# yzGuu830/efficient-speech-codec

Hardware: AMD Instinct MI355X
Metric: audio-seconds/sec encode+decode, ESC-Base 9kbps 3s@16kHz (higher is better)
Workload: dtype f32 (fp32 storage and accumulation everywhere; the K = C contractions of the MLPs, of the attention's Q / K / V projections, of PatchMerge / PatchSplit and of the de-embedding run on the fp16 matrix cores with every fp32 operand split into two fp16 terms under power-of-two scales (range-safe by cons

## Files before the change

efficient-speech-codec_amd/csrc/fused_attn.h:

```cpp
#pragma once
#include <hip/hip_runtime.h>
#include <type_traits>
#include "gemm_engine.h"
#include "gemm_bf16.h"
#include "split_terms.h"

namespace escx {

constexpr int attn_x3_ks(int CP) { return (CP + 31) / 32; }
constexpr int attn_x3_tf(int CP, int NT = 3) { return NT * attn_x3_ks(CP) > CP / 16 ? NT * attn_x3_ks(CP) : CP / 16; }
__device__ __forceinline__ void attn_split3(const float (&v)[8], bf16x8& t0, bf16x8& t1, bf16x8& t2) {
#pragma clang fp contract(off)
#pragma unroll
    for (int e = 0; e < 8; ++e) {
        const __bf16 a1 = (__bf16)v[e];
        const float r1 = v[e] - (float)a1;
        const __bf16 a2 = (__bf16)r1;
        const float r2 = r1 - (float)a2;
        t0[e] = a1; t1[e] = a2; t2[e] = (__bf16)r2;
    }
}
__global__ __launch_bounds__(256) void attn_x3_pack_kernel(const f32x4* __restrict__ waf, bf16x8* __restrict__ out, bf16x8* __restrict__ tail, int n_tiles, int TPG, int KK, int KS, int TF, unsigned proj_mask, int NT = 3,
                                                           const float* __restrict__ gamma = nullptr, const float* __restrict__ beta = nullptr, int n_ln = 0, int C = 0,
                                                           const float* __restrict__ bqkv = nullptr, int n_bqkv = 0) {
    const int per_tile = (KS > KK ? KS : KK) * 64;
    const long long idx = (long long)blockIdx.x * 256 + threadIdx.x;
    if (idx >= (long long)n_tiles * per_tile) return;
    const int tile = (int)(idx / per_tile), r = (int)(idx - (long long)tile * per_tile), f = r >> 6, lane = r & 63;
    const f32x4* src = waf + (size_t)tile * KK * 64;
    bf16x8* dst = out + (size_t)tile * TF * 64;
    if ((proj_mask >> (tile % TPG)) & 1) {
        if (f < KK) {
            const f32x4 w = src[f * 64 + lane];
            if (NT == 2 && bqkv) {
                const float sc = x2_scale(reinterpret_cast<const unsigned*>(tail)[2]);
                const float v[8] = {w[0], w[1], w[2], w[3], 0.f, 0.f, 0.f, 0.f};
                bf16x8 t[2];
                split_terms<2>(v, t, sc);
                const f32x4 hi = __builtin_bit_cast(f32x4, t[0]), lo = __builtin_bit_cast(f32x4, t[1]);
                reinterpret_cast<f32x4*>(dst)[f * 64 + lane] = f32x4{hi[0], hi[1], lo[0], lo[1]};
            } else {
                reinterpret_cast<f32x4*>(dst)[f * 64 + lane] = w;
            }
        }
        return;
    }
    if (f >= KS) return;
    const int l15 = lane & 15, g = lane >> 4;
    float v[8];
#pragma unroll
    for (int e = 0; e < 8; ++e) {
        const int kk = 2 * f + (g >> 1), lgs = 2 * (g & 1) + (e >> 2);
        v[e] = kk < KK ? src[kk * 64 + 16 * lgs + l15][e & 3] : 0.f;
    }
    if (NT == 3) {
        bf16x8 t0, t1, t2;
        attn_split3(v, t0, t1, t2);
        dst[(f * 3 + 0) * 64 + lane] = t0; dst[(f * 3 + 1) * 64 + lane] = t1; dst[(f * 3 + 2) * 64 + lane] = t2;
    } else {
        const float sc = x2_scale(*reinterpret_cast<const unsigned*>(tail));
        bf16x8 t[2];
        split_terms<2>(v, t, sc);
        dst[(f * 2 + 0) * 64 + lane] = t[0]; dst[(f * 2 + 1) * 64 + lane] = t[1];
        if (idx == 0) {
            const float bx = gamma ? ln_out_bound(gamma, beta, n_ln, C) : 0.f;
            const float sx = gamma ? act_pow2_scale(bx) : 1.0f;
            float so = 1.0f;
            const unsigned* mxs = reinterpret_cast<const unsigned*>(tail);
            if (bqkv && gamma) {
                float mb = 0.f;
                for (int i = 0; i < n_bqkv; ++i) mb = fmaxf(mb, fabsf(bqkv[i]));
                so = act_pow2_scale((float)C * __uint_as_float(mxs[1]) * bx + mb);
            }
            float* o = reinterpret_cast<float*>(tail + 1); o[0] = (1.0f / sc) * (1.0f / sx); o[1] = sc * sx; o[2] = sx; o[3] = so;
            if (bqkv) { o[4] = (1.0f / x2_scale(mxs[2])) * (1.0f / so); o[5] = 0.f; o[6] = 0.f; o[7] = 0.f; }
        }
    }
}

struct AttnArgs {
    const float* src;
    float* dst;
    const float* gamma; const float* beta;
    const f32x4* wf;
    const float* bqkv;
    const float* bias_tab;
    const float* bproj;
    const int* map;
    int slots, tokens, n_windows, nWh, nWw, shifted, C, n_groups;
    float scale, eps;
    int GS; float* partial; int rows;
    unsigned long long* trace;
    float* tape_xn; float* tape_qkv; float* tape_o; int ldq, ldo, hdp, nH;
    const void* x3_wf;
    const float* x3_scale;
};

__device__ __forceinline__ f32x4 window_shift_mask(int l15, int lg, bool lastH, bool lastW) {
    const int qh = l15 >> 2, qw = l15 & 3;
    const int labq = 3 * (lastH ? (qh < 2 ? 1 : 2) : 0) + (lastW ? (qw < 2 ? 1 : 2) : 0);
    const int labkh = 3 * (lastH ? (lg < 2 ? 1 : 2) : 0);
    f32x4 m;
#pragma unroll
    for (int r = 0; r < 4; ++r) {
        const int labk = labkh + (lastW ? (r < 2 ? 1 : 2) : 0);
        m[r] = (labk != labq) ? -100.0f : 0.0f;
    }
    return m;
}

__device__ __forceinline__ f32x4 window_softmax(f32x4 s, f32x4 bias_row, f32x4 shift_mask, bool shifted) {
    s += bias_row;
    if (shifted) s += shift_mask;
    float mx = fmaxf(fmaxf(s[0], s[1]), fmaxf(s[2], s[3]));
    mx = max_groups(mx);
    const float ml = -mx * 1.44269504088896341f;
    f32x4 p;
#pragma unroll
    for (int r = 0; r < 4; ++r) p[r] = __builtin_amdgcn_exp2f(fmaf(s[r], 1.44269504088896341f, ml));
    float den = (p[0] + p[1]) + (p[2] + p[3]);
    den = sum_groups(den);
    const float inv = __builtin_amdgcn_rcpf(den);
#pragma unroll
    for (int r = 0; r < 4; ++r) p[r] *= inv;
    return p;
}

#ifndef ESCX_ATTN_OCC3
#define ESCX_ATTN_OCC3 160
#endif
template <int CP, int TMW> constexpr int attn_min_waves() { return (CP * TMW <= 96) ? 4 : ((CP * TMW <= ESCX_ATTN_OCC3) ? 3 : ((CP * TMW <= 192) ? 2 : 1)); }

template <int CP, int TMW, bool X3> constexpr int attn_min_waves_x() { return !X3 ? attn_min_waves<CP, TMW>() : ((CP * TMW <= 96) ? 3 : ((CP * TMW <= 160) ? 2 : 1)); }

template <int CP, int MODE, int TMW, int NW, bool X3, int NT> constexpr int attn_min_waves_f() { return (X3 && NT == 2 && NW == 8 && MODE == 0 && TMW == 1 && CP <= 96) ? 4 : attn_min_waves_x<CP, TMW, X3>(); }

template <int CP, int MODE, int UT, int TMW, int NW, bool TAPE = false, bool X3 = false, int NT = 3>
__global__ __launch_bounds__(64 * NW, (attn_min_waves_f<CP, MODE, TMW, NW, X3, NT>())) void attn_fused_kernel(AttnArgs a) {
    static_assert(!X3 || !TAPE, "the split-operand form exists for the plain inference instantiations");
    static_assert(NT == 3 || (NT == 2 && X3), "two fp16 terms: the split-operand instantiations");
#ifdef ESCX_ATTN_PRIO
    __builtin_amdgcn_s_setprio(ESCX_ATTN_PRIO);
#endif
    constexpr int KK = CP / 16;
    constexpr int TPG = (MODE == 2) ? 8 : 4;
    constexpr int NB = (MODE == 2) ? 6 : 3;
    static_assert(TPG % UT == 0, "stage size must divide the tiles of a head group");
    constexpr int KS = attn_x3_ks(CP);
    constexpr int TF = X3 ? attn_x3_tf(CP, NT) : KK;
    __shared__ f32x4 wbuf_static[X3 ? 1 : 2 * UT * KK * 64];
    extern __shared__ __attribute__((aligned(16))) f32x4 wbuf_dyn[];
    f32x4* const wbuf0 = X3 ? wbuf_dyn : wbuf_static;

    const int lane = threadIdx.x & 63;
    const int l15 = lane & 15, lg = lane >> 4;
    const int wave = __builtin_amdgcn_readfirstlane(threadIdx.x >> 6);
    const int GS = a.GS > 1 ? a.GS : 1;
    const int wgb = blockIdx.x / GS, gs = blockIdx.x - wgb * GS;
    const int g0 = gs * (a.n_groups / GS), g1 = g0 + a.n_groups / GS;
    const int win0 = (wgb * NW + wave) * TMW;
    const int n_stages = (g1 - g0) * (TPG / UT);
    const f32x4* wfb = (X3 ? reinterpret_cast<const f32x4*>(a.x3_wf) : a.wf) + (size_t)g0 * TPG * TF * 64;

    constexpr int NP = UT * TF, NPW = (NP + NW - 1) / NW;
    const f32x4* dma_src = wfb + lane;
    f32x4* dma_dst = wbuf0;
    int slot = 0;
    auto dma_slot = [&]() {
        if (slot < NPW) {
            int c = wave + slot * NW;
            if (NP % NW != 0) c = min(c, NP - 1);
            __builtin_amdgcn_global_load_lds((const void*)(dma_src + c * 64), (__attribute__((address_space(3))) void*)(dma_dst + c * 64), 16, 0, 0);
        }
        ++slot;
    };
#pragma unroll
    for (int i = 0; i < NPW; ++i) dma_slot();

    const int nW = a.nWh * a.nWw;
    f32x4 xf[X3 ? 1 : TMW][X3 ? 1 : KK];
    bf16x8 xs[X3 ? TMW : 1][NT][X3 ? KS : 1];
    float x2_dn = 1.f, x2_up = 1.f, x2_sx = 1.f, x2_so = 1.f;
    if constexpr (NT == 2) { x2_dn = a.x3_scale[0]; x2_up = a.x3_scale[1]; x2_sx = a.x3_scale[2]; x2_so = a.x3_scale[3]; }
    int tok[TMW];
    bool lastH[TMW], lastW[TMW];
#pragma unroll
    for (int t = 0; t < TMW; ++t) {
        const int win = win0 + t;
        tok[t] = -1; lastH[t] = false; lastW[t] = false;
        if (win < a.n_windows) {
            const int b = win / nW, wloc = win - b * nW;
            const int wh = wloc / a.nWw, ww = wloc - wh * a.nWw;
            lastH[t] = (wh == a.nWh - 1); lastW[t] = (ww == a.nWw - 1);
            const int tk = a.map[wloc * 16 + l15];
            if (tk >= 0) tok[t] = b * a.tokens + tk;
        }
        if constexpr (X3) {
            const float* xrow = a.src + (size_t)(tok[t] < 0 ? 0 : tok[t]) * CP;
            float xv[KS][8];
            float s = 0.f;
#pragma unroll
            for (int ks = 0; ks < KS; ++ks) {
                const int c0 = 32 * ks + 8 * lg;
                f32x4 v0 = zero4(), v1 = zero4();
                if (c0 < CP) { v0 = ld4(xrow + c0); v1 = ld4(xrow + c0 + 4); }
                if (tok[t] < 0) { v0 = zero4(); v1 = zero4(); }
#pragma unroll
                for (int e = 0; e < 4; ++e) { xv[ks][e] = v0[e]; xv[ks][4 + e] = v1[e]; s += v0[e]; s += v1[e]; }
            }
            s = sum_groups(s);
            const float mean = s / (float)a.C;
            float v = 0.f;
#pragma unroll
            for (int ks = 0; ks < KS; ++ks)
#pragma unroll
                for (int e = 0; e < 8; ++e) { const float d = xv[ks][e] - mean; v += d * d; }
            v = sum_groups(v) - (float)(32 * KS - a.C) * mean * mean;
            const float rstd = 1.0f / sqrtf(v / (float)a.C + a.eps);
#pragma unroll
            for (int ks = 0; ks < KS; ++ks) {
                const int c0 = 32 * ks + 8 * lg;
                f32x4 g0v = zero4(), g1v = zero4(), b0v = zero4(), b1v = zero4();
// ... 151 lines not shown
#pragma unroll
        for (int t = 0; t < TMW; ++t) { out[t] = init; o2[t] = zero4(); }
#pragma unroll
        for (int kk = 0; kk < KK; ++kk) {
            const f32x4 w = next_frag();
            if ((kk & 1) == 0) dma_pinned();
#pragma unroll
            for (int r = 0; r < 4; ++r)
#pragma unroll
                for (int t = 0; t < TMW; ++t) {
                    if (TMW == 1 && (r & 1)) o2[t] = __builtin_amdgcn_mfma_f32_16x16x4f32(w[r], xf[t][kk][r], o2[t], 0, 0, 0);
                    else out[t] = __builtin_amdgcn_mfma_f32_16x16x4f32(w[r], xf[t][kk][r], out[t], 0, 0, 0);
                }
            ESCX_SGB_MFMA(4 * TMW);
        }
        if (TMW == 1) out[0] += o2[0];
    };
    auto gemm_x_rows = [&](f32x4* out, f32x4 init) {
        if constexpr (X3) { gemm_x3(out, init, true); return; }
        f32x4 o2[TMW];
#pragma unroll
        for (int t = 0; t < TMW; ++t) { out[t] = init; o2[t] = zero4(); }
#pragma unroll
        for (int kk = 0; kk < KK; ++kk) {
            const f32x4 w = next_frag();
            if ((kk & 1) == 0) dma_pinned();
#pragma unroll
            for (int r = 0; r < 4; ++r)
#pragma unroll
                for (int t = 0; t < TMW; ++t) {
                    if (TMW == 1 && (r & 1)) o2[t] = __builtin_amdgcn_mfma_f32_16x16x4f32(xf[t][kk][r], w[r], o2[t], 0, 0, 0);
                    else out[t] = __builtin_amdgcn_mfma_f32_16x16x4f32(xf[t][kk][r], w[r], out[t], 0, 0, 0);
                }
            ESCX_SGB_MFMA(4 * TMW);
        }
        if (TMW == 1) out[0] += o2[0];
    };
    auto proj_accumulate = [&](const f32x4* o) {
        const f32x4* tb = wb + (size_t)(((tile - 1) % UT) * TF) * 64;
        if constexpr (X3 && NT == 2) {
            bf16x8 os[TMW][2];
#pragma unroll
            for (int t = 0; t < TMW; ++t) {
                const float v8[8] = {o[t][0], o[t][1], o[t][2], o[t][3], 0.f, 0.f, 0.f, 0.f};
                split_terms<2>(v8, os[t], x2_so);
            }
#pragma unroll
            for (int to = 0; to < KK; to += 2) {
                const f32x4 w = tb[to * 64], wn = (to + 1 < KK) ? tb[(to + 1) * 64] : zero4();
                dma_pinned();
                const bf16x8 wh = __builtin_bit_cast(bf16x8, f32x4{w[0], w[1], 0.f, 0.f}), wl = __builtin_bit_cast(bf16x8, f32x4{w[2], w[3], 0.f, 0.f});
                const bf16x8 wnh = __builtin_bit_cast(bf16x8, f32x4{wn[0], wn[1], 0.f, 0.f}), wnl = __builtin_bit_cast(bf16x8, f32x4{wn[2], wn[3], 0.f, 0.f});
#define ESCX_PJ2(WH, WL, TO) _Pragma("unroll") for (int t = 0; t < TMW; ++t) acc[TO][t] = mma_x<2>(WH, os[t][1], acc[TO][t]); \
                             _Pragma("unroll") for (int t = 0; t < TMW; ++t) acc[TO][t] = mma_x<2>(WL, os[t][0], acc[TO][t]); \
                             _Pragma("unroll") for (int t = 0; t < TMW; ++t) acc[TO][t] = mma_x<2>(WH, os[t][0], acc[TO][t]);
                if (to + 1 < KK) {
#pragma unroll
                    for (int t = 0; t < TMW; ++t) { acc[to][t] = mma_x<2>(wh, os[t][1], acc[to][t]); acc[to + 1][t] = mma_x<2>(wnh, os[t][1], acc[to + 1][t]); }
#pragma unroll
                    for (int t = 0; t < TMW; ++t) { acc[to][t] = mma_x<2>(wl, os[t][0], acc[to][t]); acc[to + 1][t] = mma_x<2>(wnl, os[t][0], acc[to + 1][t]); }
#pragma unroll
                    for (int t = 0; t < TMW; ++t) { acc[to][t] = mma_x<2>(wh, os[t][0], acc[to][t]); acc[to + 1][t] = mma_x<2>(wnh, os[t][0], acc[to + 1][t]); }
                } else { ESCX_PJ2(wh, wl, to) }
#undef ESCX_PJ2
            }
            return;
        }
#pragma unroll
        for (int to = 0; to < KK; to += 2) {
            f32x4 w, wn = zero4();
            if constexpr (X3) { w = tb[to * 64]; if (to + 1 < KK) wn = tb[(to + 1) * 64]; }
            else { w = next_frag(); if (to + 1 < KK) wn = next_frag(); }
            dma_pinned();
#pragma unroll
            for (int r = 0; r < 4; ++r)
#pragma unroll
                for (int t = 0; t < TMW; ++t) {
                    acc[to][t] = __builtin_amdgcn_mfma_f32_16x16x4f32(w[r], o[t][r], acc[to][t], 0, 0, 0);
                    if (to + 1 < KK) acc[to + 1][t] = __builtin_amdgcn_mfma_f32_16x16x4f32(wn[r], o[t][r], acc[to + 1][t], 0, 0, 0);
                }
            if constexpr (!X3) { if (to + 1 < KK) ESCX_SGB_MFMA(8 * TMW); else ESCX_SGB_MFMA(4 * TMW); }
        }
    };
    struct GroupConst { f32x4 b[4]; f32x4 bt0, bt1; float bv0, bv1; };
    auto load_consts = [&](int g) -> GroupConst {
        GroupConst c;
        const float* bg = a.bqkv + (size_t)g * NB * 16;
        if constexpr (MODE != 2) {
            c.b[0] = ld4(bg + 4 * lg); c.b[1] = ld4(bg + 16 + 4 * lg); c.b[2] = zero4(); c.b[3] = zero4();
            c.bv0 = bg[32 + l15]; c.bv1 = 0.f;
            const float* bt = a.bias_tab + (size_t)(MODE == 1 ? 2 * g : g) * 256 + l15 * 16 + 4 * lg;
            c.bt0 = ld4(bt); c.bt1 = (MODE == 1) ? ld4(bt + 256) : zero4();
            ESCX_SGB_VMEM(MODE == 1 ? 5 : 4);
        } else {
#pragma unroll
            for (int i = 0; i < 4; ++i) c.b[i] = ld4(bg + i * 16 + 4 * lg);
            c.bv0 = bg[4 * 16 + l15]; c.bv1 = bg[5 * 16 + l15];
            c.bt0 = ld4(a.bias_tab + (size_t)g * 256 + l15 * 16 + 4 * lg); c.bt1 = zero4();
            ESCX_SGB_VMEM(7);
        }
        return c;
    };
    auto pin_consts = [&](GroupConst& c) {
        asm volatile("" : "+v"(c.b[0]), "+v"(c.b[1]), "+v"(c.bt0), "+v"(c.bv0));
        if constexpr (MODE == 1) asm volatile("" : "+v"(c.bt1));
        if constexpr (MODE == 2) asm volatile("" : "+v"(c.b[2]), "+v"(c.b[3]), "+v"(c.bv1));
    };

#ifdef ESCX_ATTN_TRACE
    unsigned long long tr[8] = {0, 0, 0, 0, 0, 0, 0, 0};
#define ESCX_TS(var) unsigned long long var; { __builtin_amdgcn_sched_barrier(0); var = __builtin_amdgcn_s_memtime(); __builtin_amdgcn_sched_barrier(0); }
    ESCX_TS(t_begin)
#else
#define ESCX_TS(var)
#endif
    f32x4 shmask[TMW];
#pragma unroll
    for (int t = 0; t < TMW; ++t) shmask[t] = window_shift_mask(l15, lg, lastH[t], lastW[t]);
    GroupConst cur = load_consts(g0);
    for (int g = g0; g < g1; ++g) {
        tile = 0;
        ESCX_TS(t0)
        begin_tile();
        pin_consts(cur);
        const GroupConst nxt = load_consts(min(g + 1, g1 - 1));
        ESCX_TS(t1)
        f32x4 q[TMW], k[TMW], vt[TMW], o[TMW];
        if constexpr (MODE != 2) {
            gemm_w_rows(q, cur.b[0]);
#pragma unroll
            for (int t = 0; t < TMW; ++t) q[t] *= a.scale;
            begin_tile();
            gemm_w_rows(k, cur.b[1]);
            if constexpr (TAPE) {
                tape_rows(a.tape_qkv, a.ldq, 0, g, 0, q);
                tape_rows(a.tape_qkv, a.ldq, a.nH * a.hdp, g, 0, k);
            }
            ESCX_TS(t2)
            f32x4 p0[TMW], p1[TMW];
#pragma unroll
            for (int t = 0; t < TMW; ++t) {
                if constexpr (MODE == 0) {
                    f32x4 s = zero4();
#pragma unroll
                    for (int r = 0; r < 4; ++r) s = __builtin_amdgcn_mfma_f32_16x16x4f32(k[t][r], q[t][r], s, 0, 0, 0);
                    p0[t] = window_softmax(s, cur.bt0, shmask[t], a.shifted);
                } else {
                    f32x4 sa = zero4(), sb = zero4();
#pragma unroll
                    for (int r = 0; r < 4; ++r) {
                        sa = __builtin_amdgcn_mfma_f32_16x16x4f32(k[t][r], lg < 2 ? q[t][r] : 0.f, sa, 0, 0, 0);
                        sb = __builtin_amdgcn_mfma_f32_16x16x4f32(k[t][r], lg < 2 ? 0.f : q[t][r], sb, 0, 0, 0);
                    }
                    p0[t] = window_softmax(sa, cur.bt0, shmask[t], a.shifted);
                    p1[t] = window_softmax(sb, cur.bt1, shmask[t], a.shifted);
                }
            }
            ESCX_SGB_MFMA((MODE == 0 ? 4 : 8) * TMW);
            ESCX_TS(t3)
            begin_tile();
            gemm_x_rows(vt, f32x4{cur.bv0, cur.bv0, cur.bv0, cur.bv0});
            ESCX_TS(t4)
#pragma unroll
            for (int t = 0; t < TMW; ++t) {
                f32x4 oa = zero4();
#pragma unroll
                for (int r = 0; r < 4; ++r) oa = __builtin_amdgcn_mfma_f32_16x16x4f32(vt[t][r], p0[t][r], oa, 0, 0, 0);
                if constexpr (MODE == 1) {
                    f32x4 ob = zero4();
#pragma unroll
                    for (int r = 0; r < 4; ++r) ob = __builtin_amdgcn_mfma_f32_16x16x4f32(vt[t][r], p1[t][r], ob, 0, 0, 0);
                    o[t] = lg < 2 ? oa : ob;
                } else {
                    o[t] = oa;
                }
            }
            ESCX_SGB_MFMA((MODE == 0 ? 4 : 8) * TMW);
            if constexpr (TAPE) {
                tape_cols(a.tape_qkv, a.ldq, 2 * a.nH * a.hdp, g, 0, vt);
                tape_rows(a.tape_o, a.ldo, 0, g, 0, o);
            }
            ESCX_TS(t5)
            begin_tile();
            proj_accumulate(o);
            ESCX_TS(t6)
#ifdef ESCX_ATTN_TRACE
            tr[0] += t1 - t0; tr[1] += t2 - t1; tr[2] += t3 - t2; tr[3] += t4 - t3; tr[4] += t5 - t4; tr[5] += t6 - t5;
#endif
        } else {
            f32x4 s[TMW];
#pragma unroll
            for (int t = 0; t < TMW; ++t) s[t] = zero4();
#pragma unroll
            for (int half = 0; half < 2; ++half) {
                if (half) begin_tile();
                gemm_w_rows(q, cur.b[2 * half]);
#pragma unroll
                for (int t = 0; t < TMW; ++t) q[t] *= a.scale;
                begin_tile();
                gemm_w_rows(k, cur.b[2 * half + 1]);
                if constexpr (TAPE) {
                    tape_rows(a.tape_qkv, a.ldq, 0, g, half, q);
// ... 400 lines not shown
```

efficient-speech-codec_amd/csrc/fused_swin.hip:

```cpp
#include "fused_attn.h"
#include "fused_mlp.h"
#include "fused_mlp_x3.h"
#include <atomic>
#include "fused_rowgemm.h"
#include "fused_deembed.h"
#include "launchers.h"

namespace escx {

template <int CP, int TM>
static void launch_mlp(const MlpArgs& a, hipStream_t s) {
    const int waves = (a.M + 16 * TM - 1) / (16 * TM);
    ESCX_LAUNCH((mlp_fused_kernel<CP, TM>), dim3((waves + 3) / 4), dim3(256), 0, s, a);
}

template <int CP, int TM, int NW>
static void launch_mlp_lds(const MlpArgs& a, hipStream_t s) {
    const int rows = 16 * TM * NW;
    const int hs = a.HS > 1 ? a.HS : 1;
    ESCX_LAUNCH((mlp_fused_lds_kernel<CP, TM, NW>), dim3(((a.M + rows - 1) / rows) * hs), dim3(64 * NW), 0, s, a);
}

template <int CP>
static int launch_mlp_lds_variant(int variant, const MlpArgs& a, hipStream_t s) {
// ... 133 lines not shown
}

int mlp_x3(float* x, int M, int C, int Cp, const float* gamma, const float* beta, const float* b1, const float* b2, const void* image, int hiddenP, int nw, int* hs_io, float* partial,
           hipStream_t s, const MlpSplit* split, int nt, float* out) {
    if (!image || hiddenP % 32 || (nt != 2 && nt != 3)) return -1;
    if (out && (split || (hs_io && *hs_io > 1))) return -1;
    if (split) {
        if ((hs_io && *hs_io > 1) || !split->wf || !(Cp == 80 || Cp == 96 || Cp == 144)) return ESCX_COMB_UNSUPPORTED;
        MlpArgs a{};
        a.x = x; a.gamma = gamma; a.beta = beta; a.b1 = b1; a.b2 = b2; a.M = M; a.C = C; a.HT = hiddenP / 16; a.eps = 1e-5f; a.HS = 1; a.x3_w = image;
        a.sp_wf = reinterpret_cast<const f32x4*>(split->wf); a.sp_gamma = split->gamma; a.sp_beta = split->beta; a.sp_out = split->out;
        a.sp_NT = split->NT; a.sp_H = split->H; a.sp_W = split->W; a.sp_C2p = split->C2p;
        switch (Cp) {
#define ESCX_X3S_CASE(CPV) case CPV: if (nt == 2) { if (nw == 8) launch_mlp_x3_split<CPV, 8, 2>(a, s); else launch_mlp_x3_split<CPV, 4, 2>(a, s); } \
                           else { if (nw == 8) launch_mlp_x3_split<CPV, 8>(a, s); else launch_mlp_x3_split<CPV, 4>(a, s); } return 0;
            ESCX_X3S_CASE(80) ESCX_X3S_CASE(96) ESCX_X3S_CASE(144)
#undef ESCX_X3S_CASE
        }
        return ESCX_COMB_UNSUPPORTED;
    }
    int hs = hs_io ? *hs_io : 1;
    if (hs > 1 && (!partial || (hiddenP / 32) % hs)) hs = 1;
    if (hs_io) *hs_io = hs;
    MlpArgs a{};
    a.x = x; a.gamma = gamma; a.beta = beta; a.b1 = b1; a.b2 = b2; a.M = M; a.C = C; a.HT = hiddenP / 16; a.eps = 1e-5f; a.HS = hs; a.partial = partial; a.x3_w = image; a.out = out;
#define ESCX_X3_CASE(CPV) case CPV: if (nt == 2) { if (nw == 8) launch_mlp_x3<CPV, 8, 2>(a, s); else launch_mlp_x3<CPV, 4, 2>(a, s); } \
                          else { if (nw == 8) launch_mlp_x3<CPV, 8>(a, s); else launch_mlp_x3<CPV, 4>(a, s); } return 0;
    switch (Cp) {
        ESCX_X3_CASE(48) ESCX_X3_CASE(80) ESCX_X3_CASE(96) ESCX_X3_CASE(144) ESCX_X3_CASE(192) ESCX_X3_CASE(384)
        default: return -1;
    }
#undef ESCX_X3_CASE
}


template <int KP, int SEGS>
static int launch_rowgemm(const RowGemmArgs& a, hipStream_t s) {
    if (a.x3_wf) {
        if constexpr (KP == 96 || KP == 160 || KP == 192 || KP == 288 || KP == 384 || KP == 144 || KP == 80) {
            constexpr int KSx = (KP + 31) / 32, TFx = 3 * KSx, UTx = 36 / TFx >= 4 ? 4 : (36 / TFx >= 2 ? 2 : 1);
            constexpr int TMx = KP <= 96 ? 2 : 1, NWx = 4;
            auto kern = rowgemm_x3_kernel<KP, SEGS, TMx, NWx, UTx>;
            auto kern2 = rowgemm_x3_kernel<KP, SEGS, TMx, NWx, UTx, 2>;
            constexpr int lds = 2 * UTx * TFx * 1024, lds2 = 2 * UTx * 2 * KSx * 1024;
            if constexpr (lds > 48 * 1024) {
                static std::atomic<unsigned> done{0};
                int dev = 0; (void)hipGetDevice(&dev);
                const unsigned bit = 1u << (dev & 31);
                if (!(done.load(std::memory_order_relaxed) & bit)) {
                    (void)hipFuncSetAttribute((const void*)kern, hipFuncAttributeMaxDynamicSharedMemorySize, lds);
                    (void)hipFuncSetAttribute((const void*)kern2, hipFuncAttributeMaxDynamicSharedMemorySize, lds2);
                    done.fetch_or(bit, std::memory_order_relaxed);
                }
            }
            if (a.x3_scale) ESCX_LAUNCH(kern2, dim3((a.M + 16 * TMx * NWx - 1) / (16 * TMx * NWx), 1), dim3(64 * NWx), lds2, s, a);
            else ESCX_LAUNCH(kern, dim3((a.M + 16 * TMx * NWx - 1) / (16 * TMx * NWx), 1), dim3(64 * NWx), lds, s, a);
            return 0;
        }
    }
    constexpr int KK = KP / 16;
    constexpr int UT = KK <= 6 ? 4 : (KK <= 12 ? 2 : 1);
    constexpr int TM = KP <= 192 ? 2 : 1;
    constexpr int NW = 4;
    const int rows = 16 * TM * NW;
    RowGemmArgs b = a;
    b.nt_chunk = (a.NT + UT - 1) / UT * UT;
    const int chunks = (a.NT + b.nt_chunk - 1) / b.nt_chunk;
    ESCX_LAUNCH((rowgemm_fused_kernel<KP, SEGS, TM, NW, UT>), dim3((a.M + rows - 1) / rows, chunks), dim3(64 * NW), 0, s, b);
    return 0;
}

size_t rowgemm_x3_bytes(int KP, int Np) { return (size_t)(Np / 16) * 3 * ((KP + 31) / 32) * 1024 + 32; }
static char* rowgemm_x3_trailer(const void* image, int KP, int Np) { return reinterpret_cast<char*>(const_cast<void*>(image)) + rowgemm_x3_bytes(KP, Np) - 32; }
int rowgemm_x3_pack(const float* wf, void* image, int KP, int Np, hipStream_t s, int nt, const float* gamma, const float* beta, int C) {
    const int KK = KP / 16, KS = (KP + 31) / 32, NT = Np / 16;
    const long long total = (long long)NT * (KS > KK ? KS : KK) * 64;
    if (nt == 2) {
        unsigned* mx = reinterpret_cast<unsigned*>(rowgemm_x3_trailer(image, KP, Np));
        (void)hipMemsetAsync(mx, 0, 16, s);
        const long long n = (long long)NT * KK * 64 * 4;
        ESCX_LAUNCH(absmax_bits_kernel, dim3((unsigned)std::min<long long>(256, (n + 255) / 256)), dim3(256), 0, s, wf, n, mx);
    }
    ESCX_LAUNCH(attn_x3_pack_kernel, dim3((unsigned)((total + 255) / 256)), dim3(256), 0, s, reinterpret_cast<const f32x4*>(wf), reinterpret_cast<bf16x8*>(image),
                       reinterpret_cast<bf16x8*>(rowgemm_x3_trailer(image, KP, Np)), NT, 1, KK, KS, (nt == 2 ? 2 : 3) * KS, 0u, nt == 2 ? 2 : 3, gamma, beta, KP, C, (const float*)nullptr, 0);
    return 0;
}

int rowgemm_fused(int segs, const float* x, float* out, const float* gamma, const float* beta, const float* wf, const int* map, int M,
                  int rows_per_clip, int src_rows_per_clip, int C, int Cp, int Np, int split, int H, int W, int C2p, hipStream_t s,
                  const void* x3_wf, int x3_nt) {
    const int KP = segs * Cp;
    RowGemmArgs a{x, out, gamma, beta, reinterpret_cast<const f32x4*>(wf), map, M, rows_per_clip, src_rows_per_clip, C, Cp, Np / 16,
                  split, H, W, C2p, 1e-5f, Np / 16, x3_wf,
                  (x3_wf && x3_nt == 2) ? reinterpret_cast<const float*>(rowgemm_x3_trailer(x3_wf, KP, Np) + 16) : nullptr};
    if (segs == 1) {
        switch (KP) {
            case 16: return launch_rowgemm<16, 1>(a, s);
            case 48: return launch_rowgemm<48, 1>(a, s);
            case 80: return launch_rowgemm<80, 1>(a, s);
            case 96: return launch_rowgemm<96, 1>(a, s);
            case 144: return launch_rowgemm<144, 1>(a, s);
            case 192: return launch_rowgemm<192, 1>(a, s);
            case 384: return launch_rowgemm<384, 1>(a, s);
            default: return -1;
        }
    }
    switch (KP) {
        case 32: return launch_rowgemm<32, 2>(a, s);
        case 96: return launch_rowgemm<96, 2>(a, s);
        case 160: return launch_rowgemm<160, 2>(a, s);
        case 192: return launch_rowgemm<192, 2>(a, s);
        case 288: return launch_rowgemm<288, 2>(a, s);
        case 384: return launch_rowgemm<384, 2>(a, s);
        default: return -1;
    }
}

size_t deembed7_x2_image_bytes(int Cp) { return Cp == 48 ? deembed7_x2_bytes(Cp) : 0; }
int deembed7_x2_pack(const float* wfrag, void* image, int Cp, hipStream_t s) {
    if (Cp != 48) return -1;
    const int nsteps = de2_steps(Cp);
    unsigned* mx = reinterpret_cast<unsigned*>(reinterpret_cast<char*>(image) + deembed7_x2_bytes(Cp) - 32);
    if (hipMemsetAsync(mx, 0, 32, s) != hipSuccess) return -1;
    const long long n = (long long)49 * (Cp / 16) * 64 * 4;
    ESCX_LAUNCH(absmax_bits_kernel, dim3((unsigned)std::min<long long>(256, (n + 255) / 256)), dim3(256), 0, s, wfrag, n, mx);
    ESCX_LAUNCH(deembed7_x2_pack_kernel, dim3((nsteps * 64 + 255) / 256), dim3(256), 0, s, reinterpret_cast<const f32x4*>(wfrag), reinterpret_cast<bf16x8*>(image), Cp, nsteps);
    return 0;
}

int deembed7_fused(const float* tok, int B, int H, int W, int Cp, const float* wfrag, const float* bias, float* out, int pf, int pt,
                   int in_dim, int Fp, hipStream_t s, const void* x2_image) {
    DeembedArgs a{tok, reinterpret_cast<const f32x4*>(wfrag), bias, out, B, H, W, pf, pt, in_dim, Fp, in_dim * pf * pt};
    if (a.n_out > 16) return -1;
    const int grid = B * ((H + 7) / 8) * ((W + 31) / 32);
    if (x2_image && Cp == 48) {
        auto kern = deembed7_x2_kernel<48>;
        constexpr int lds = 2 * 14 * 38 * (48 + 8) * 2 + 2 * 8 * 2 * 1024;
        static std::atomic<unsigned> done{0};
        int dev = 0; (void)hipGetDevice(&dev);
        const unsigned bit = 1u << (dev & 31);
        if (!(done.load(std::memory_order_relaxed) & bit)) { (void)hipFuncSetAttribute((const void*)kern, hipFuncAttributeMaxDynamicSharedMemorySize, lds); done.fetch_or(bit, std::memory_order_relaxed); }
        ESCX_LAUNCH(kern, dim3(grid), dim3(512), lds, s, a, reinterpret_cast<const bf16x8*>(x2_image));
        return 0;
    }
    switch (Cp) {
        case 16: ESCX_LAUNCH(deembed7_kernel<16>, dim3(grid), dim3(512), 0, s, a); return 0;
        case 32: ESCX_LAUNCH(deembed7_kernel<32>, dim3(grid), dim3(512), 0, s, a); return 0;
        case 48: ESCX_LAUNCH(deembed7_kernel<48>, dim3(grid), dim3(512), 0, s, a); return 0;
        default: return -1;
    }
}

template <int CP, int MODE, int NW>
static int launch_attn(const AttnArgs& a, hipStream_t s) {
    constexpr int UT = CP <= 96 ? 4 : (CP <= 192 ? 2 : 1);
    constexpr int TMW = attn_windows_per_wave(CP);
    const int per_block = TMW * NW;
    const int gs = a.GS > 1 ? a.GS : 1;
    if (a.tape_qkv) {
        if constexpr (CP == 16 || CP == 48 || CP == 80 || CP == 96) {
            if (gs == 1) {
                ESCX_LAUNCH((attn_fused_kernel<CP, MODE, UT, TMW, NW, true>), dim3((a.n_windows + per_block - 1) / per_block), dim3(64 * NW), 0, s, a);
                return 0;
            }
        }
        return ESCX_COMB_UNSUPPORTED;
    }
    if constexpr ((CP == 48 && MODE == 0) || (CP == 80 && (MODE == 0 || MODE == 2)) || (CP == 96 && MODE != 2) || (CP == 144 && MODE != 2) || (CP == 192 && MODE == 1)) {
        if (a.x3_wf) {
            auto kern = attn_fused_kernel<CP, MODE, UT, TMW, NW, false, true>;
            auto kern2 = attn_fused_kernel<CP, MODE, UT, TMW, NW, false, true, 2>;
            constexpr int lds = 2 * UT * attn_x3_tf(CP) * 1024, lds2 = 2 * UT * attn_x3_tf(CP, 2) * 1024;
            if constexpr (lds > 48 * 1024) {
                static std::atomic<unsigned> done{0};
                int dev = 0; (void)hipGetDevice(&dev);
                const unsigned bit = 1u << (dev & 31);
                if (!(done.load(std::memory_order_relaxed) & bit)) {
                    (void)hipFuncSetAttribute((const void*)kern, hipFuncAttributeMaxDynamicSharedMemorySize, lds);
                    (void)hipFuncSetAttribute((const void*)kern2, hipFuncAttributeMaxDynamicSharedMemorySize, lds2);
                    done.fetch_or(bit, std::memory_order_relaxed);
                }
            }
            if (a.x3_scale) ESCX_LAUNCH(kern2, dim3(((a.n_windows + per_block - 1) / per_block) * gs), dim3(64 * NW), lds2, s, a);
            else ESCX_LAUNCH(kern, dim3(((a.n_windows + per_block - 1) / per_block) * gs), dim3(64 * NW), lds, s, a);
            return 0;
        }
    }
    ESCX_LAUNCH((attn_fused_kernel<CP, MODE, UT, TMW, NW>), dim3(((a.n_windows + per_block - 1) / per_block) * gs), dim3(64 * NW), 0, s, a);
    return 0;
}

template <int CP>
static int launch_attn_cp(int mode, int nw, const AttnArgs& a, hipStream_t s) {
    if (nw == 8) {
        switch (mode) {
            case 0: return launch_attn<CP, 0, 8>(a, s);
            case 1: return launch_attn<CP, 1, 8>(a, s);
            case 2: return launch_attn<CP, 2, 8>(a, s);
        }
    } else {
        switch (mode) {
            case 0: return launch_attn<CP, 0, 4>(a, s);
            case 1: return launch_attn<CP, 1, 4>(a, s);
            case 2: return launch_attn<CP, 2, 4>(a, s);
        }
    }
    return -1;
}

template <int CP, int NW>
static int launch_attn_packed(const AttnArgs& a, hipStream_t s) {
    constexpr int UT = CP <= 96 ? 4 : (CP <= 192 ? 2 : 1);
    const int pairs = (a.n_windows + 1) / 2;
    const int gs = a.GS > 1 ? a.GS : 1;
    if constexpr (CP == 384 && NW == 4) {
        if (a.x3_wf) {
            auto kern = attn_packed_kernel<CP, UT, NW, true>;
            auto kern2 = attn_packed_kernel<CP, UT, NW, true, 2>;
            constexpr int lds = 2 * UT * attn_x3_tf(CP) * 1024, lds2 = 2 * UT * attn_x3_tf(CP, 2) * 1024;
            static std::atomic<unsigned> done{0};
            int dev = 0; (void)hipGetDevice(&dev);
            const unsigned bit = 1u << (dev & 31);
            if (!(done.load(std::memory_order_relaxed) & bit)) {
                (void)hipFuncSetAttribute((const void*)kern, hipFuncAttributeMaxDynamicSharedMemorySize, lds);
                (void)hipFuncSetAttribute((const void*)kern2, hipFuncAttributeMaxDynamicSharedMemorySize, lds2);
                done.fetch_or(bit, std::memory_order_relaxed);
            }
            if (a.x3_scale) ESCX_LAUNCH(kern2, dim3(((pairs + NW - 1) / NW) * gs), dim3(64 * NW), lds2, s, a);
            else ESCX_LAUNCH(kern, dim3(((pairs + NW - 1) / NW) * gs), dim3(64 * NW), lds, s, a);
            return 0;
        }
    }
    ESCX_LAUNCH((attn_packed_kernel<CP, UT, NW>), dim3(((pairs + NW - 1) / NW) * gs), dim3(64 * NW), 0, s, a);
    return 0;
}

size_t attn_x3_bytes(int Cp, int mode, int n_groups) { return (size_t)n_groups * (mode == 2 ? 8 : 4) * attn_x3_tf(Cp) * 1024 + 48; }
static char* attn_x3_trailer(const void* image, int Cp, int mode, int n_groups) { return reinterpret_cast<char*>(const_cast<void*>(image)) + attn_x3_bytes(Cp, mode, n_groups) - 48; }

int attn_x3_pack(const float* waf, void* image, int Cp, int mode, int n_groups, hipStream_t s, int nt, const float* gamma, const float* beta, int C, const float* bqkv) {
    const int KK = Cp / 16, KS = attn_x3_ks(Cp), TF = attn_x3_tf(Cp, nt == 2 ? 2 : 3), TPG = mode == 2 ? 8 : 4;
    const unsigned proj_mask = mode == 2 ? ((1u << 5) | (1u << 7)) : (1u << 3);
    const int n_tiles = n_groups * TPG;
    (void)hipMemsetAsync(image, 0, attn_x3_bytes(Cp, mode, n_groups), s);
    const long long total = (long long)n_tiles * (KS > KK ? KS : KK) * 64;
    if (nt == 2) {
        unsigned* mx = reinterpret_cast<unsigned*>(attn_x3_trailer(image, Cp, mode, n_groups));
        const long long n = (long long)n_tiles * KK * 64 * 4;
        const unsigned all = (1u << TPG) - 1, vmask = mode == 2 ? ((1u << 4) | (1u << 6)) : (1u << 2);
        const dim3 grid((unsigned)std::min<long long>(256, (n + 255) / 256));
        ESCX_LAUNCH(absmax_tiles_bits_kernel, grid, dim3(256), 0, s, waf, n, KK * 256, TPG, all & ~proj_mask, mx);
        ESCX_LAUNCH(absmax_tiles_bits_kernel, grid, dim3(256), 0, s, waf, n, KK * 256, TPG, vmask, mx + 1);
        ESCX_LAUNCH(absmax_tiles_bits_kernel, grid, dim3(256), 0, s, waf, n, KK * 256, TPG, proj_mask, mx + 2);
    }
    ESCX_LAUNCH(attn_x3_pack_kernel, dim3((unsigned)((total + 255) / 256)), dim3(256), 0, s, reinterpret_cast<const f32x4*>(waf), reinterpret_cast<bf16x8*>(image),
                       reinterpret_cast<bf16x8*>(attn_x3_trailer(image, Cp, mode, n_groups)), n_tiles, TPG, KK, KS, TF, proj_mask, nt == 2 ? 2 : 3, gamma, beta, Cp, C, bqkv, n_groups * (mode == 2 ? 6 : 3) * 16);
    return 0;
}

int attn_fused(const float* src, float* dst, int Cp, int C, int mode, int n_groups, const float* gamma, const float* beta,
               const float* wf, const float* bqkv, const float* bias_tab, const float* bproj, const int* map, int slots, int tokens,
               int n_windows, int nWh, int nWw, int shifted, float scale, int nw, int* gs_io, float* partial, int rows, hipStream_t s,
               const AttnTape* tape, const void* x3_wf, int x3_nt) {
    int gs = gs_io ? *gs_io : 1;
    if (gs > 1 && (!partial || n_groups % gs)) gs = 1;
    if (gs_io) *gs_io = gs;
    AttnArgs a{src, dst, gamma, beta, reinterpret_cast<const f32x4*>(wf), bqkv, bias_tab, bproj, map, slots, tokens, n_windows,
               nWh, nWw, shifted, C, n_groups, scale, 1e-5f, gs, partial, rows, g_mlp_trace,
               tape ? tape->xn : nullptr, tape ? tape->qkv : nullptr, tape ? tape->o : nullptr, tape ? tape->ldq : 0, tape ? tape->ldo : 0,
               tape ? tape->hdp : 0, tape ? tape->nH : 0, tape ? nullptr : x3_wf,
               (!tape && x3_wf && x3_nt == 2) ? reinterpret_cast<const float*>(attn_x3_trailer(x3_wf, Cp, mode, n_groups) + 16) : nullptr};
    if (tape && nw < 0) return ESCX_COMB_UNSUPPORTED;
    if (nw < 0) {
        nw = -nw;
        if (mode == 0) {
#define ESCX_PACK(CPV) case CPV: return nw == 8 ? launch_attn_packed<CPV, 8>(a, s) : launch_attn_packed<CPV, 4>(a, s);
            switch (Cp) { ESCX_PACK(64) ESCX_PACK(96) ESCX_PACK(128) ESCX_PACK(192) ESCX_PACK(256) ESCX_PACK(384) default: break; }
#undef ESCX_PACK
        }
    }
    switch (Cp) {
        case 16: return launch_attn_cp<16>(mode, nw, a, s);
        case 32: return launch_attn_cp<32>(mode, nw, a, s);
        case 48: return launch_attn_cp<48>(mode, nw, a, s);
        case 64: return launch_attn_cp<64>(mode, nw, a, s);
        case 80: return launch_attn_cp<80>(mode, nw, a, s);
        case 96: return launch_attn_cp<96>(mode, nw, a, s);
        case 128: return launch_attn_cp<128>(mode, nw, a, s);
        case 144: return launch_attn_cp<144>(mode, nw, a, s);
        case 192: return launch_attn_cp<192>(mode, nw, a, s);
        case 256: return launch_attn_cp<256>(mode, nw, a, s);
        case 384: return launch_attn_cp<384>(mode, nw, a, s);
        default: return -1;
    }
}

}
```

Before: 12000.

## Pair head groups so the attention output projection uses full-width fp16 MFMA operands

Adds a paired-head-group variant of the two-term split-operand attention kernel. Two heads' outputs (or the two halves of a mode-2 group) are packed into one 8-wide fp16 operand, and the pack kernel interleaves the projection weights to match. This lets one MFMA sequence serve the output projection of both heads and fills the fp16 K dimension that was half padded before. In exchange it adds a new packed weight layout, pairing constraints on group counts and the split factor, a higher occupancy bound for mode 1, and more code paths (unsupported pairings return an error).

```diff
diff --git a/efficient-speech-codec_amd/csrc/fused_attn.h b/efficient-speech-codec_amd/csrc/fused_attn.h
--- a/efficient-speech-codec_amd/csrc/fused_attn.h
+++ b/efficient-speech-codec_amd/csrc/fused_attn.h
@@ -22,13 +22,16 @@
 }
 __global__ __launch_bounds__(256) void attn_x3_pack_kernel(const f32x4* __restrict__ waf, bf16x8* __restrict__ out, bf16x8* __restrict__ tail, int n_tiles, int TPG, int KK, int KS, int TF, unsigned proj_mask, int NT = 3,
                                                            const float* __restrict__ gamma = nullptr, const float* __restrict__ beta = nullptr, int n_ln = 0, int C = 0,
-                                                           const float* __restrict__ bqkv = nullptr, int n_bqkv = 0) {
+                                                           const float* __restrict__ bqkv = nullptr, int n_bqkv = 0, int pair = 0) {
     const int per_tile = (KS > KK ? KS : KK) * 64;
     const long long idx = (long long)blockIdx.x * 256 + threadIdx.x;
     if (idx >= (long long)n_tiles * per_tile) return;
     const int tile = (int)(idx / per_tile), r = (int)(idx - (long long)tile * per_tile), f = r >> 6, lane = r & 63;
     const f32x4* src = waf + (size_t)tile * KK * 64;
-    bf16x8* dst = out + (size_t)tile * TF * 64;
+    int dtile = tile, unit = 0, ph = 0;
+    if (pair == 1) { const int grp = tile / TPG, tt = tile % TPG; unit = grp >> 1; ph = grp & 1; dtile = unit * 8 + 3 * ph + tt; }
+    else if (pair == 2) { const int tt = tile % TPG; unit = tile / TPG; ph = tt == 7; dtile = unit * 8 + (tt == 6 ? 5 : tt); }
+    bf16x8* dst = out + (size_t)dtile * TF * 64;
     if ((proj_mask >> (tile % TPG)) & 1) {
         if (f < KK) {
             const f32x4 w = src[f * 64 + lane];
@@ -38,6 +41,12 @@
                 bf16x8 t[2];
                 split_terms<2>(v, t, sc);
                 const f32x4 hi = __builtin_bit_cast(f32x4, t[0]), lo = __builtin_bit_cast(f32x4, t[1]);
+                if (pair) {
+                    const int KH = (KK + 1) / 2, hf = f >= KH, j = f - hf * KH;
+                    float2* d = reinterpret_cast<float2*>(out + (size_t)(unit * 8 + 6 + hf) * TF * 64);
+                    d[((2 * j) * 64 + lane) * 2 + ph] = float2{hi[0], hi[1]};
+                    d[((2 * j + 1) * 64 + lane) * 2 + ph] = float2{lo[0], lo[1]};
+                } else
                 reinterpret_cast<f32x4*>(dst)[f * 64 + lane] = f32x4{hi[0], hi[1], lo[0], lo[1]};
             } else {
                 reinterpret_cast<f32x4*>(dst)[f * 64 + lane] = w;
@@ -133,11 +142,14 @@
 
 template <int CP, int TMW, bool X3> constexpr int attn_min_waves_x() { return !X3 ? attn_min_waves<CP, TMW>() : ((CP * TMW <= 96) ? 3 : ((CP * TMW <= 160) ? 2 : 1)); }
 
-template <int CP, int MODE, int TMW, int NW, bool X3, int NT> constexpr int attn_min_waves_f() { return (X3 && NT == 2 && NW == 8 && MODE == 0 && TMW == 1 && CP <= 96) ? 4 : attn_min_waves_x<CP, TMW, X3>(); }
-
-template <int CP, int MODE, int UT, int TMW, int NW, bool TAPE = false, bool X3 = false, int NT = 3>
-__global__ __launch_bounds__(64 * NW, (attn_min_waves_f<CP, MODE, TMW, NW, X3, NT>())) void attn_fused_kernel(AttnArgs a) {
+template <int CP, int MODE, int TMW, int NW, bool X3, int NT, bool PAIR = false> constexpr int attn_min_waves_f() {
+    return (X3 && NT == 2 && TMW == 1 && CP <= 96 && ((NW == 8 && MODE == 0) || (PAIR && MODE == 1))) ? 4 : attn_min_waves_x<CP, TMW, X3>();
+}
+
+template <int CP, int MODE, int UT, int TMW, int NW, bool TAPE = false, bool X3 = false, int NT = 3, bool PAIR = false>
+__global__ __launch_bounds__(64 * NW, (attn_min_waves_f<CP, MODE, TMW, NW, X3, NT, PAIR>())) void attn_fused_kernel(AttnArgs a) {
     static_assert(!X3 || !TAPE, "the split-operand form exists for the plain inference instantiations");
+    static_assert(!PAIR || (X3 && NT == 2), "paired head groups: the two-term instantiations (attn_x3_pack_kernel)");
     static_assert(NT == 3 || (NT == 2 && X3), "two fp16 terms: the split-operand instantiations");
 #ifdef ESCX_ATTN_PRIO
     __builtin_amdgcn_s_setprio(ESCX_ATTN_PRIO);
@@ -455,6 +467,37 @@
             if constexpr (!X3) { if (to + 1 < KK) ESCX_SGB_MFMA(8 * TMW); else ESCX_SGB_MFMA(4 * TMW); }
         }
     };
+    auto proj_pair = [&](const f32x4* oa, const f32x4* ob) {
+        if constexpr (PAIR) {
+            bf16x8 os[TMW][2];
+#pragma unroll
+            for (int t = 0; t < TMW; ++t) {
+                const float v8[8] = {oa[t][0], oa[t][1], oa[t][2], oa[t][3], ob[t][0], ob[t][1], ob[t][2], ob[t][3]};
+                split_terms<2>(v8, os[t], x2_so);
+            }
+            constexpr int KH = (KK + 1) / 2;
+#pragma unroll
+            for (int hf = 0; hf < 2; ++hf) {
+                begin_tile();
+                const bf16x8* tb = reinterpret_cast<const bf16x8*>(wb) + (size_t)(((tile - 1) % UT) * TF) * 64;
+                const int base = hf * KH, n = hf ? KK - KH : KH;
+#pragma unroll
+                for (int j = 0; j < n; j += 2) {
+                    const bool two = j + 1 < n;
+                    const bf16x8 wh = tb[(2 * j) * 64], wl = tb[(2 * j + 1) * 64];
+                    const bf16x8 wnh = tb[(two ? 2 * j + 2 : 2 * j) * 64], wnl = tb[(two ? 2 * j + 3 : 2 * j + 1) * 64];
+                    dma_pinned();
+                    const int to = base + j, tn = two ? to + 1 : to;
+#pragma unroll
+                    for (int t = 0; t < TMW; ++t) { acc[to][t] = mma_x<2>(wh, os[t][1], acc[to][t]); if (two) acc[tn][t] = mma_x<2>(wnh, os[t][1], acc[tn][t]); }
+#pragma unroll
+                    for (int t = 0; t < TMW; ++t) { acc[to][t] = mma_x<2>(wl, os[t][0], acc[to][t]); if (two) acc[tn][t] = mma_x<2>(wnl, os[t][0], acc[tn][t]); }
+#pragma unroll
+                    for (int t = 0; t < TMW; ++t) { acc[to][t] = mma_x<2>(wh, os[t][0], acc[to][t]); if (two) acc[tn][t] = mma_x<2>(wnh, os[t][0], acc[tn][t]); }
+                }
+            }
+        }
+    };
     struct GroupConst { f32x4 b[4]; f32x4 bt0, bt1; float bv0, bv1; };
     auto load_consts = [&](int g) -> GroupConst {
         GroupConst c;
@@ -491,6 +534,112 @@
 #pragma unroll
     for (int t = 0; t < TMW; ++t) shmask[t] = window_shift_mask(l15, lg, lastH[t], lastW[t]);
     GroupConst cur = load_consts(g0);
+    if constexpr (PAIR && MODE != 2) {
+        for (int g = g0; g < g1; g += 2) {
+            tile = 0;
+            f32x4 op[2][TMW];
+#pragma unroll
+            for (int h = 0; h < 2; ++h) {
+                ESCX_TS(t0)
+                begin_tile();
+                pin_consts(cur);
+                const GroupConst nxt = load_consts(min(g + h + 1, g1 - 1));
+                ESCX_TS(t1)
+                f32x4 q[TMW], k[TMW], vt[TMW], p0[TMW], p1[TMW];
+                gemm_w_rows(q, cur.b[0]);
+#pragma unroll
+                for (int t = 0; t < TMW; ++t) q[t] *= a.scale;
+                begin_tile();
+                gemm_w_rows(k, cur.b[1]);
+                ESCX_TS(t2)
+#pragma unroll
+                for (int t = 0; t < TMW; ++t) {
+                    if constexpr (MODE == 0) {
+                        f32x4 s = zero4();
+#pragma unroll
+                        for (int r = 0; r < 4; ++r) s = __builtin_amdgcn_mfma_f32_16x16x4f32(k[t][r], q[t][r], s, 0, 0, 0);
+                        p0[t] = window_softmax(s, cur.bt0, shmask[t], a.shifted);
+                    } else {
+                        f32x4 sa = zero4(), sb = zero4();
+#pragma unroll
+                        for (int r = 0; r < 4; ++r) {
+                            sa = __builtin_amdgcn_mfma_f32_16x16x4f32(k[t][r], lg < 2 ? q[t][r] : 0.f, sa, 0, 0, 0);
+                            sb = __builtin_amdgcn_mfma_f32_16x16x4f32(k[t][r], lg < 2 ? 0.f : q[t][r], sb, 0, 0, 0);
+                        }
+                        p0[t] = window_softmax(sa, cur.bt0, shmask[t], a.shifted);
+                        p1[t] = window_softmax(sb, cur.bt1, shmask[t], a.shifted);
+                    }
+                }
+                ESCX_TS(t3)
+                begin_tile();
+                gemm_x_rows(vt, f32x4{cur.bv0, cur.bv0, cur.bv0, cur.bv0});
+                ESCX_TS(t4)
+#pragma unroll
+                for (int t = 0; t < TMW; ++t) {
+                    f32x4 oa = zero4();
+#pragma unroll
+                    for (int r = 0; r < 4; ++r) oa = __builtin_amdgcn_mfma_f32_16x16x4f32(vt[t][r], p0[t][r], oa, 0, 0, 0);
+                    if constexpr (MODE == 1) {
+                        f32x4 ob = zero4();
+#pragma unroll
+                        for (int r = 0; r < 4; ++r) ob = __builtin_amdgcn_mfma_f32_16x16x4f32(vt[t][r], p1[t][r], ob, 0, 0, 0);
+                        op[h][t] = lg < 2 ? oa : ob;
+                    } else {
+                        op[h][t] = oa;
+                    }
+                }
+                ESCX_TS(t5)
+#ifdef ESCX_ATTN_TRACE
+                tr[0] += t1 - t0; tr[1] += t2 - t1; tr[2] += t3 - t2; tr[3] += t4 - t3; tr[4] += t5 - t4;
+#endif
+                cur = nxt;
+            }
+            ESCX_TS(t6)
+            proj_pair(op[0], op[1]);
+            ESCX_TS(t7)
+#ifdef ESCX_ATTN_TRACE
+            tr[5] += t7 - t6;
+#endif
+        }
+    } else if constexpr (PAIR) {
+        for (int g = g0; g < g1; ++g) {
+            tile = 0;
+            begin_tile();
+            pin_consts(cur);
+            const GroupConst nxt = load_consts(min(g + 1, g1 - 1));
+            f32x4 q[TMW], k[TMW], vt[TMW], s[TMW], p[TMW], op[2][TMW];
+#pragma unroll
+            for (int t = 0; t < TMW; ++t) s[t] = zero4();
+#pragma unroll
+            for (int half = 0; half < 2; ++half) {
+                if (half) begin_tile();
+                gemm_w_rows(q, cur.b[2 * half]);
+#pragma unroll
+                for (int t = 0; t < TMW; ++t) q[t] *= a.scale;
+                begin_tile();
+                gemm_w_rows(k, cur.b[2 * half + 1]);
+#pragma unroll
+                for (int t = 0; t < TMW; ++t)
+#pragma unroll
+                    for (int r = 0; r < 4; ++r) s[t] = __builtin_amdgcn_mfma_f32_16x16x4f32(k[t][r], q[t][r], s[t], 0, 0, 0);
+            }
+#pragma unroll
+            for (int t = 0; t < TMW; ++t) p[t] = window_softmax(s[t], cur.bt0, shmask[t], a.shifted);
+#pragma unroll
+            for (int half = 0; half < 2; ++half) {
+                begin_tile();
+                { const float bvh = half ? cur.bv1 : cur.bv0; gemm_x_rows(vt, f32x4{bvh, bvh, bvh, bvh}); }
+#pragma unroll
+                for (int t = 0; t < TMW; ++t) {
+                    op[half][t] = zero4();
+#pragma unroll
+                    for (int r = 0; r < 4; ++r) op[half][t] = __builtin_amdgcn_mfma_f32_16x16x4f32(vt[t][r], p[t][r], op[half][t], 0, 0, 0);
+                }
+            }
+            proj_pair(op[0], op[1]);
+            cur = nxt;
+        }
+    } else
     for (int g = g0; g < g1; ++g) {
         tile = 0;
         ESCX_TS(t0)
diff --git a/efficient-speech-codec_amd/csrc/fused_swin.hip b/efficient-speech-codec_amd/csrc/fused_swin.hip
--- a/efficient-speech-codec_amd/csrc/fused_swin.hip
+++ b/efficient-speech-codec_amd/csrc/fused_swin.hip
@@ -239,7 +239,7 @@
         ESCX_LAUNCH(absmax_bits_kernel, dim3((unsigned)std::min<long long>(256, (n + 255) / 256)), dim3(256), 0, s, wf, n, mx);
     }
     ESCX_LAUNCH(attn_x3_pack_kernel, dim3((unsigned)((total + 255) / 256)), dim3(256), 0, s, reinterpret_cast<const f32x4*>(wf), reinterpret_cast<bf16x8*>(image),
-                       reinterpret_cast<bf16x8*>(rowgemm_x3_trailer(image, KP, Np)), NT, 1, KK, KS, (nt == 2 ? 2 : 3) * KS, 0u, nt == 2 ? 2 : 3, gamma, beta, KP, C, (const float*)nullptr, 0);
+                       reinterpret_cast<bf16x8*>(rowgemm_x3_trailer(image, KP, Np)), NT, 1, KK, KS, (nt == 2 ? 2 : 3) * KS, 0u, nt == 2 ? 2 : 3, gamma, beta, KP, C, (const float*)nullptr, 0, 0);
     return 0;
 }
 
@@ -308,8 +308,13 @@
     }
 }
 
+static constexpr bool attn_x3_fused(int Cp, int mode) {
+    return (Cp == 48 && mode == 0) || (Cp == 80 && (mode == 0 || mode == 2)) || (Cp == 96 && mode != 2) || (Cp == 144 && mode != 2) || (Cp == 192 && mode == 1);
+}
+static int attn_x3_pairing(int Cp, int mode, int n_groups) { return (!attn_x3_fused(Cp, mode) || Cp < 80) ? 0 : (mode == 2 ? 2 : (n_groups % 2 == 0 ? 1 : 0)); }
+
 template <int CP, int MODE, int NW>
-static int launch_attn(const AttnArgs& a, hipStream_t s) {
+static int launch_attn(const AttnArgs& a, hipStream_t s, bool pair) {
     constexpr int UT = CP <= 96 ? 4 : (CP <= 192 ? 2 : 1);
     constexpr int TMW = attn_windows_per_wave(CP);
     const int per_block = TMW * NW;
@@ -323,7 +328,7 @@
         }
         return ESCX_COMB_UNSUPPORTED;
     }
-    if constexpr ((CP == 48 && MODE == 0) || (CP == 80 && (MODE == 0 || MODE == 2)) || (CP == 96 && MODE != 2) || (CP == 144 && MODE != 2) || (CP == 192 && MODE == 1)) {
+    if constexpr (attn_x3_fused(CP, MODE)) {
         if (a.x3_wf) {
             auto kern = attn_fused_kernel<CP, MODE, UT, TMW, NW, false, true>;
             auto kern2 = attn_fused_kernel<CP, MODE, UT, TMW, NW, false, true, 2>;
@@ -338,6 +343,20 @@
                     done.fetch_or(bit, std::memory_order_relaxed);
                 }
             }
+            if constexpr (CP >= 80) {
+                if (a.x3_scale && pair) {
+                    auto kern2p = attn_fused_kernel<CP, MODE, UT, TMW, NW, false, true, 2, true>;
+                    if constexpr (lds2 > 48 * 1024) {
+                        static std::atomic<unsigned> donep{0};
+                        int dev = 0; (void)hipGetDevice(&dev);
+                        const unsigned bit = 1u << (dev & 31);
+                        if (!(donep.load(std::memory_order_relaxed) & bit)) { (void)hipFuncSetAttribute((const void*)kern2p, hipFuncAttributeMaxDynamicSharedMemorySize, lds2); donep.fetch_or(bit, std::memory_order_relaxed); }
+                    }
+                    ESCX_LAUNCH(kern2p, dim3(((a.n_windows + per_block - 1) / per_block) * gs), dim3(64 * NW), lds2, s, a);
+                    return 0;
+                }
+            }
+            if (pair) return -1;
             if (a.x3_scale) ESCX_LAUNCH(kern2, dim3(((a.n_windows + per_block - 1) / per_block) * gs), dim3(64 * NW), lds2, s, a);
             else ESCX_LAUNCH(kern, dim3(((a.n_windows + per_block - 1) / per_block) * gs), dim3(64 * NW), lds, s, a);
             return 0;
@@ -348,18 +367,18 @@
 }
 
 template <int CP>
-static int launch_attn_cp(int mode, int nw, const AttnArgs& a, hipStream_t s) {
+static int launch_attn_cp(int mode, int nw, const AttnArgs& a, hipStream_t s, bool pair) {
     if (nw == 8) {
         switch (mode) {
-            case 0: return launch_attn<CP, 0, 8>(a, s);
-            case 1: return launch_attn<CP, 1, 8>(a, s);
-            case 2: return launch_attn<CP, 2, 8>(a, s);
+            case 0: return launch_attn<CP, 0, 8>(a, s, pair);
+            case 1: return launch_attn<CP, 1, 8>(a, s, pair);
+            case 2: return launch_attn<CP, 2, 8>(a, s, pair);
         }
     } else {
         switch (mode) {
-            case 0: return launch_attn<CP, 0, 4>(a, s);
-            case 1: return launch_attn<CP, 1, 4>(a, s);
-            case 2: return launch_attn<CP, 2, 4>(a, s);
+            case 0: return launch_attn<CP, 0, 4>(a, s, pair);
+            case 1: return launch_attn<CP, 1, 4>(a, s, pair);
+            case 2: return launch_attn<CP, 2, 4>(a, s, pair);
         }
     }
     return -1;
@@ -398,6 +417,7 @@
 int attn_x3_pack(const float* waf, void* image, int Cp, int mode, int n_groups, hipStream_t s, int nt, const float* gamma, const float* beta, int C, const float* bqkv) {
     const int KK = Cp / 16, KS = attn_x3_ks(Cp), TF = attn_x3_tf(Cp, nt == 2 ? 2 : 3), TPG = mode == 2 ? 8 : 4;
     const unsigned proj_mask = mode == 2 ? ((1u << 5) | (1u << 7)) : (1u << 3);
+    const int pair = nt == 2 ? attn_x3_pairing(Cp, mode, n_groups) : 0;
     const int n_tiles = n_groups * TPG;
     (void)hipMemsetAsync(image, 0, attn_x3_bytes(Cp, mode, n_groups), s);
     const long long total = (long long)n_tiles * (KS > KK ? KS : KK) * 64;
@@ -411,7 +431,7 @@
         ESCX_LAUNCH(absmax_tiles_bits_kernel, grid, dim3(256), 0, s, waf, n, KK * 256, TPG, proj_mask, mx + 2);
     }
     ESCX_LAUNCH(attn_x3_pack_kernel, dim3((unsigned)((total + 255) / 256)), dim3(256), 0, s, reinterpret_cast<const f32x4*>(waf), reinterpret_cast<bf16x8*>(image),
-                       reinterpret_cast<bf16x8*>(attn_x3_trailer(image, Cp, mode, n_groups)), n_tiles, TPG, KK, KS, TF, proj_mask, nt == 2 ? 2 : 3, gamma, beta, Cp, C, bqkv, n_groups * (mode == 2 ? 6 : 3) * 16);
+                       reinterpret_cast<bf16x8*>(attn_x3_trailer(image, Cp, mode, n_groups)), n_tiles, TPG, KK, KS, TF, proj_mask, nt == 2 ? 2 : 3, gamma, beta, Cp, C, bqkv, n_groups * (mode == 2 ? 6 : 3) * 16, pair);
     return 0;
 }
 
@@ -421,6 +441,8 @@
                const AttnTape* tape, const void* x3_wf, int x3_nt) {
     int gs = gs_io ? *gs_io : 1;
     if (gs > 1 && (!partial || n_groups % gs)) gs = 1;
+    const int pairing = (!tape && x3_wf && x3_nt == 2) ? attn_x3_pairing(Cp, mode, n_groups) : 0;
+    if (pairing == 1 && (n_groups / gs) % 2) gs = 1;
     if (gs_io) *gs_io = gs;
     AttnArgs a{src, dst, gamma, beta, reinterpret_cast<const f32x4*>(wf), bqkv, bias_tab, bproj, map, slots, tokens, n_windows,
                nWh, nWw, shifted, C, n_groups, scale, 1e-5f, gs, partial, rows, g_mlp_trace,
@@ -437,19 +459,19 @@
         }
     }
     switch (Cp) {
-        case 16: return launch_attn_cp<16>(mode, nw, a, s);
-        case 32: return launch_attn_cp<32>(mode, nw, a, s);
-        case 48: return launch_attn_cp<48>(mode, nw, a, s);
-        case 64: return launch_attn_cp<64>(mode, nw, a, s);
-        case 80: return launch_attn_cp<80>(mode, nw, a, s);
-        case 96: return launch_attn_cp<96>(mode, nw, a, s);
-        case 128: return launch_attn_cp<128>(mode, nw, a, s);
-        case 144: return launch_attn_cp<144>(mode, nw, a, s);
-        case 192: return launch_attn_cp<192>(mode, nw, a, s);
-        case 256: return launch_attn_cp<256>(mode, nw, a, s);
-        case 384: return launch_attn_cp<384>(mode, nw, a, s);
-        default: return -1;
-    }
-}
-
-}
+        case 16: return launch_attn_cp<16>(mode, nw, a, s, pairing != 0);
+        case 32: return launch_attn_cp<32>(mode, nw, a, s, pairing != 0);
+        case 48: return launch_attn_cp<48>(mode, nw, a, s, pairing != 0);
+        case 64: return launch_attn_cp<64>(mode, nw, a, s, pairing != 0);
+        case 80: return launch_attn_cp<80>(mode, nw, a, s, pairing != 0);
+        case 96: return launch_attn_cp<96>(mode, nw, a, s, pairing != 0);
+        case 128: return launch_attn_cp<128>(mode, nw, a, s, pairing != 0);
+        case 144: return launch_attn_cp<144>(mode, nw, a, s, pairing != 0);
+        case 192: return launch_attn_cp<192>(mode, nw, a, s, pairing != 0);
+        case 256: return launch_attn_cp<256>(mode, nw, a, s, pairing != 0);
+        case 384: return launch_attn_cp<384>(mode, nw, a, s, pairing != 0);
+        default: return -1;
+    }
+}
+
+}
```

After: 12330 (median of 6 runs). +2.7%, better.
